# uncertaintyhub/chsimpy

Measured on AMD Instinct MI355X. Metric: timesteps/sec at N=4096 fp64; achieved HBM GB/s vs MI355X peak, higher is better.
Workload: dtype f64; 1 GPU; N=4096 fp64 Cahn-Hilliard timestep loop (BASELINE.json configs[2] at N=4096), U_init = 0.875 + 0.00875*(PCG64(2023).random - 0.5), kappa_tilde=0.0002989112919661156, full_sim; N=4096, engine=fast, ensemble=single run

## Files before the change

### chsimpy_amd/csrc/chs_fast_core.h

```cpp
#pragma once
#include <hip/hip_runtime.h>
#include <type_traits>
#include "chs_cx.h"

template <typename T_, int N_, int G_, int THREADS_, int R0_, int RA_, int RB_, int RL_, int PAD1_, int PAD2_,
          int PADL_, int WPS_, int CT_ = THREADS_ / G_, int XPAIR_ = -1>
struct FCfg {
  using T = T_;
  using V = Cx<T_>;
  static constexpr int N = N_;
  static constexpr int M = N_ / 2;
  static constexpr int G = G_;
  static constexpr int E = M / G_;
  static constexpr int R0 = R0_, RA = RA_, RB = RB_, RL = RL_;
  static constexpr int R2 = RL_;
  static constexpr int S1 = R0_;
  static constexpr int S2A = R0_ * RA_;
  static constexpr int SL = R0_ * RA_ * RB_;
  static constexpr int S2 = SL;
  static constexpr int L1 = M / R0_;
  static constexpr int L2 = L1 / RA_;
  static constexpr int L3 = L2 / RB_;
  static constexpr int NP0 = E / (2 * R0_);
  static constexpr int NBA = E / RA_;
// ... 318 lines not shown
  }
}
template <class C, bool WR, int PART>
__device__ __forceinline__ void mv_a_out(typename C::V* z, typename C::T* scr, int l) {
#pragma unroll
  for (int ib = 0; ib < C::NBA; ++ib) {
    const int id = l + C::G * ib;
    const int kap = id % C::S1, mm = id / C::S1;
#pragma unroll
    for (int k = 0; k < C::RA; ++k) {
      if constexpr (C::RB > 1) xfer<C, WR, PART>(z[ib * C::RA + k], scr, (kap + C::S1 * k) * C::P2 + mm);
      else xfer<C, WR, PART>(z[ib * C::RA + k], scr, mm * C::PL + kap + C::S1 * k);
    }
  }
}
template <class C, bool WR, int PART>
__device__ __forceinline__ void mv_b_in(typename C::V* z, typename C::T* scr, int l) {
#pragma unroll
  for (int ib = 0; ib < C::NBB; ++ib) {
    const int id = l + C::G * ib;
    const int kap = id % C::S2A, mm = id / C::S2A;
#pragma unroll
    for (int j = 0; j < C::RB; ++j) xfer<C, WR, PART>(z[ib * C::RB + j], scr, kap * C::P2 + mm + C::L3 * j);
  }
}
template <class C, bool WR, int PART>
__device__ __forceinline__ void mv_b_out(typename C::V* z, typename C::T* scr, int l) {
#pragma unroll
  for (int ib = 0; ib < C::NBB; ++ib) {
    const int id = l + C::G * ib;
    const int kap = id % C::S2A, mm = id / C::S2A;
#pragma unroll
    for (int k = 0; k < C::RB; ++k) xfer<C, WR, PART>(z[ib * C::RB + k], scr, mm * C::PL + kap + C::S2A * k);
  }
}
template <class C, bool WR, int PART>
__device__ __forceinline__ void mv_last(typename C::V* z, typename C::T* scr, int l) {
#pragma unroll
  for (int q = 0; q < C::NP2; ++q) {
    int k1, k2; bool sp;
    Own<C>::last_pair(l, q, k1, k2, sp);
#pragma unroll
    for (int j = 0; j < C::RL; ++j) {
      xfer<C, WR, PART>(z[(q * 2 + 0) * C::RL + j], scr, j * C::PL + k1);
      xfer<C, WR, PART>(z[(q * 2 + 1) * C::RL + j], scr, j * C::PL + k2);
    }
  }
}

#define CHS_EXCHANGE(WRITER, READER)                                                   \
  do {                                                                                 \
    xsync<C>(); WRITER<C, true, 0>(z, scr, l); xsync<C>(); READER<C, false, 0>(z, scr, l);   \
    if constexpr (!C::PAIR) {                                                          \
      xsync<C>(); WRITER<C, true, 1>(z, scr, l); xsync<C>(); READER<C, false, 1>(z, scr, l); \
    }                                                                                  \
  } while (0)

template <class C, bool POW>
__device__ __forceinline__ void tw0_load(const typename C::T* tw0, int m, typename C::V* w ) {
  using T = typename C::T;
  if constexpr (!POW) {
#pragma unroll
    for (int k = 1; k < C::R0; ++k) w[k] = ldc<T>(tw0, (k - 1) * C::L1 + m);
  } else {
    w[1] = ldc<T>(tw0, m);
#pragma unroll
    for (int k = 2; k < C::R0; ++k) w[k] = cx_mul(w[k / 2], w[k - k / 2]);
  }
}

template <class C, bool TW0POW = false>
__device__ __forceinline__ void fwd_passes(typename C::V* z, typename C::T* scr, const FTables<typename C::T>& tb, int l) {
  using T = typename C::T;
  using V = typename C::V;
#pragma unroll
  for (int q = 0; q < C::NP0; ++q) {
    const int m1 = l + C::G * q;
#pragma unroll
    for (int b = 0; b < 2; ++b) {
      const int m = b ? (C::L1 - 1 - m1) : m1;
      V* r = z + (q * 2 + b) * C::R0;
      Dft<V, C::R0, false>::run(r);
      V w[C::R0];
      tw0_load<C, TW0POW>(tb.tw0, m, w);
#pragma unroll
      for (int k = 1; k < C::R0; ++k) r[k] = cx_mul(r[k], w[k]);
    }
  }
  if constexpr (C::RA > 1) {
    CHS_EXCHANGE(mv_pass0, mv_a_in);
    mid_fwd<C, C::S1, C::L2, C::RA, C::NBA>(z, tb.twa, l);
    if constexpr (C::RB > 1) {
      CHS_EXCHANGE(mv_a_out, mv_b_in);
      mid_fwd<C, C::S2A, C::L3, C::RB, C::NBB>(z, tb.twb, l);
      CHS_EXCHANGE(mv_b_out, mv_last);
    } else {
      CHS_EXCHANGE(mv_a_out, mv_last);
    }
  } else {
    CHS_EXCHANGE(mv_pass0, mv_last);
  }
#pragma unroll
  for (int q = 0; q < 2 * C::NP2; ++q) Dft<V, C::RL, false>::run(z + q * C::RL);
}

template <class C, bool TW0POW = false>
__device__ __forceinline__ void inv_passes(typename C::V* z, typename C::T* scr, const FTables<typename C::T>& tb, int l) {
  using T = typename C::T;
  using V = typename C::V;
#pragma unroll
  for (int q = 0; q < 2 * C::NP2; ++q) Dft<V, C::RL, true>::run(z + q * C::RL);
  if constexpr (C::RA > 1) {
    if constexpr (C::RB > 1) {
      CHS_EXCHANGE(mv_last, mv_b_out);
      mid_inv<C, C::S2A, C::L3, C::RB, C::NBB>(z, tb.twb, l);
      CHS_EXCHANGE(mv_b_in, mv_a_out);
    } else {
      CHS_EXCHANGE(mv_last, mv_a_out);
    }
    mid_inv<C, C::S1, C::L2, C::RA, C::NBA>(z, tb.twa, l);
    CHS_EXCHANGE(mv_a_in, mv_pass0);
  } else {
    CHS_EXCHANGE(mv_last, mv_pass0);
  }
#pragma unroll
  for (int q = 0; q < C::NP0; ++q) {
    const int m1 = l + C::G * q;
#pragma unroll
    for (int b = 0; b < 2; ++b) {
      const int m = b ? (C::L1 - 1 - m1) : m1;
      V* r = z + (q * 2 + b) * C::R0;
      V w[C::R0];
      tw0_load<C, TW0POW>(tb.tw0, m, w);
#pragma unroll
      for (int k = 1; k < C::R0; ++k) r[k] = cx_mulc(r[k], w[k]);
      Dft<V, C::R0, true>::run(r);
    }
  }
}

#ifndef CHS_RSTAMP
#define CHS_RSTAMP(I) do {} while (0)
#define CHS_RSTAMP1(I) do {} while (0)
#endif
struct NoFetch {};
__device__ __forceinline__ int fc_opaque(int x) {
  asm volatile("" : "+v"(x));
  __builtin_assume(x >= 0 && x < 8192);
  return x;
}

template <class C>
struct PreAll { static constexpr bool value = (C::E <= 8); };
template <class C, bool FWD, bool ADJ, bool PIPE_, class PRE, class F, class ST>
__device__ __forceinline__ void recombine(typename C::V* z, const FTables<typename C::T>& tb, int l, PRE&& pre, F&& f, ST&& st) {
  using T = typename C::T;
  using V = typename C::V;
  constexpr bool PREALL = PreAll<C>::value;
  constexpr bool PIPE = PIPE_ && !PREALL;
  constexpr int R2 = C::R2, N = C::N, M = C::M, H = R2 / 2;
  const V zero = cx_make(T(0), T(0));
#pragma unroll
  for (int q = 0; q < C::NP2; ++q) {
    V* r1 = z + (q * 2 + 0) * R2;
    V* r2 = z + (q * 2 + 1) * R2;
    const int kap = l + C::G * q;
    bool has_special = false;
    if (q == 0) has_special = (C::G < 64) || (__builtin_amdgcn_readfirstlane(l) == 0);
    if (!has_special) {
      SlotTw<T> wn;
      const int id0[5] = {kap, N - kap, M - kap, M + kap, kap};
      decltype(pre(0, id0)) pn;
      [[maybe_unused]] SlotTw<T> wv[PREALL ? R2 : 1];
      [[maybe_unused]] decltype(pre(0, id0)) pv[PREALL ? R2 : 1];
      if constexpr (PIPE) {
        wn = slot_tw<T>(tb, kap);
        pn = pre(q * R2 * 4, id0);
      }
      if constexpr (PREALL) {
#pragma unroll
        for (int k = 0; k < R2; ++k) {
          const int kk = kap + C::S2 * k;
          wv[k] = slot_tw<T>(tb, kk);
          const int idc[5] = {kk, N - kk, M - kk, M + kk, kk};
          pv[k] = pre((q * R2 + k) * 4, idc);
        }
      }
      CHS_RSTAMP1(0);
#pragma unroll
      for (int k = 0; k < R2; ++k) {
        if (k == 1) CHS_RSTAMP1(1);
        if (k == 4) CHS_RSTAMP1(2);
        const int kk = kap + C::S2 * k;
        if constexpr (PREALL) {
          wn = wv[k]; pn = pv[k];
        } else if (!PIPE) {
          wn = slot_tw<T>(tb, kk);
          const int idc[5] = {kk, N - kk, M - kk, M + kk, kk};
          pn = pre((q * R2 + k) * 4, idc);
        }
        const SlotTw<T> w = wn;
        const auto pc = pn;
        V Ya = zero, Yb = zero;
        if constexpr (FWD) slot_fwd<T>(r1[k], r2[R2 - 1 - k], w, Ya, Yb);
        const int idx[5] = {kk, N - kk, M - kk, M + kk, kk};
        f((q * R2 + k) * 4, idx, Ya, Yb, true, pc);
        if (PIPE && k + 1 < R2) {
          const int kn = fc_opaque(kap) + C::S2 * (k + 1);
          wn = slot_tw<T>(tb, kn);
          const int idn[5] = {kn, N - kn, M - kn, M + kn, kn};
          pn = pre((q * R2 + k + 1) * 4, idn);
        }
        st((q * R2 + k) * 4, idx, Ya, Yb, true);
        if constexpr (ADJ) slot_adj<T>(Ya, Yb, w, r1[k], r2[R2 - 1 - k]);
      }
      CHS_RSTAMP1(3);
    } else {
      const bool sp = (kap == 0);
      auto sel = [&](V a, V b) { return cx_make(sp ? cx_re(a) : cx_re(b), sp ? cx_im(a) : cx_im(b)); };
      auto kk_of = [&](int k) {
        const int kk_s = (k == 0) ? C::S2 : ((k < H) ? C::S2 * k : C::S2 / 2 + C::S2 * (k - H));
        return sp ? kk_s : kap + C::S2 * k;
      };
      const int kk0 = kk_of(0);
      SlotTw<T> wn;
      const int o1 = PIPE ? (sp ? 0 : kk0) : kk0, o2 = PIPE ? (sp ? M / 2 : N - kk0) : N - kk0;
      const int o3 = PIPE ? (sp ? M : M - kk0) : M - kk0, o4 = PIPE ? (sp ? 3 * (M / 2) : M + kk0) : M + kk0;
      const int id0[5] = {o1, o2, o3, o4, (PIPE && sp) ? M + 1 : kk0};
      decltype(pre(0, id0)) pn;
      SlotTw<T> whp = SlotTw<T>();
      [[maybe_unused]] SlotTw<T> wv[PREALL ? R2 : 1];
      [[maybe_unused]] decltype(pre(0, id0)) pv[PREALL ? R2 : 1];
      [[maybe_unused]] SlotTw<T> w0v = SlotTw<T>();
      [[maybe_unused]] decltype(pre(0, id0)) p0v;
      if constexpr (PIPE) {
        wn = slot_tw<T>(tb, o1);
        pn = pre(q * R2 * 4, id0);
        if (sp) whp = slot_tw<T>(tb, M / 2);
      }
      if constexpr (PREALL) {
        if (sp) {
          const int ido[5] = {0, M / 2, M, 3 * (M / 2), M + 1};
          w0v = slot_tw<T>(tb, 0); whp = slot_tw<T>(tb, M / 2);
          p0v = pre(q * R2 * 4, ido);
        }
#pragma unroll
        for (int k = 0; k < R2; ++k) {
          const int kk = kk_of(k);
          wv[k] = slot_tw<T>(tb, kk);
          const int idc[5] = {kk, N - kk, M - kk, M + kk, kk};
          pv[k] = pre((q * R2 + k) * 4, idc);
        }
      }
      CHS_RSTAMP(0);
      if (sp) {
        const int idx[5] = {0, M / 2, M, 3 * (M / 2), M + 1};
        SlotTw<T> w0, wh;
        decltype(pre(0, id0)) p0;
        if constexpr (PREALL) {
          w0 = w0v; wh = whp; p0 = p0v;
        } else if constexpr (PIPE) {
          w0 = wn; wh = whp; p0 = pn;
        } else {
          w0 = slot_tw<T>(tb, 0); wh = slot_tw<T>(tb, M / 2);
          p0 = pre(q * R2 * 4, idx);
        }
        V Ya = zero, Yb = zero;
        if constexpr (FWD) {
          V a01, a23, b01, b23;
          slot_fwd<T>(r1[0], r1[0], w0, a01, a23);
          slot_fwd<T>(r1[H], r1[H], wh, b01, b23);
          Ya = cx_make(cx_re(a01), cx_re(b01));
          Yb = cx_make(cx_re(a23), cx_im(b01));
        }
        f(q * R2 * 4, idx, Ya, Yb, true, p0);
        st(q * R2 * 4, idx, Ya, Yb, true);
        if constexpr (ADJ) {
          V ga, gz;
          slot_adj<T>(cx_make(cx_re(Ya), T(0)), cx_make(cx_re(Yb), T(0)), w0, ga, gz);
          r1[0] = cx_add(ga, gz);
          slot_adj<T>(cx_make(cx_im(Ya), cx_im(Yb)), zero, wh, ga, gz);
          r1[H] = cx_add(ga, gz);
        }
      }
      CHS_RSTAMP(1);
#pragma unroll
      for (int k = 0; k < R2; ++k) {
        if (k == 1) CHS_RSTAMP(2);
        if (k == 4) CHS_RSTAMP(3);
        const int kk = kk_of(k);
        if constexpr (PREALL) {
          wn = wv[k]; pn = pv[k];
        } else if (!PIPE) {
          wn = slot_tw<T>(tb, kk);
          const int idc[5] = {kk, N - kk, M - kk, M + kk, kk};
          pn = pre((q * R2 + k) * 4, idc);
        }
        const SlotTw<T> w = wn;
        const auto pc = pn;
        V* a_n = &r1[k]; V* b_n = &r2[R2 - 1 - k];
        V* a_s = (k < H) ? &r1[k] : &r2[k - H];
        V* b_s = (k == 0) ? &r2[R2 - 1] : ((k < H) ? &r1[R2 - k] : &r2[R2 - 1 - (k - H)]);
        V Ya = zero, Yb = zero;
        if constexpr (FWD) slot_fwd<T>(sel(*a_s, *a_n), sel(*b_s, *b_n), w, Ya, Yb);
        const int idx[5] = {kk, N - kk, M - kk, M + kk, kk};
        const bool live = (k > 0) || !sp;
        f((q * R2 + k) * 4, idx, Ya, Yb, live, pc);
        if (PIPE && k + 1 < R2) {
          const int kap_o = fc_opaque(kap);
          const int kn = sp ? kk_of(k + 1) : kap_o + C::S2 * (k + 1);
          wn = slot_tw<T>(tb, kn);
          const int idn[5] = {kn, N - kn, M - kn, M + kn, kn};
          pn = pre((q * R2 + k + 1) * 4, idn);
        }
        st((q * R2 + k) * 4, idx, Ya, Yb, live);
        if constexpr (ADJ) {
          V na, nb;
          slot_adj<T>(Ya, Yb, w, na, nb);
          if (k == 0) {
            *a_n = sel(*a_n, na);
            *b_n = sel(*b_n, nb);
          } else {
            if (k < H) {
              *a_n = na;
            } else {
              *a_s = sel(na, *a_s);
              *a_n = sel(*a_n, na);
            }
            *b_s = sel(nb, *b_s);
            *b_n = sel(*b_n, nb);
          }
        }
      }
      CHS_RSTAMP(4);
    }
  }
}

template <class C>
__device__ __forceinline__ void pack_quads(const typename C::T q1[4], const typename C::T q2[4], int q, int j, typename C::V* z) {
  constexpr int R0 = C::R0;
  z[(q * 2 + 0) * R0 + j] = cx_make(q1[0], q1[2]);
  z[(q * 2 + 1) * R0 + j] = cx_make(q2[0], q2[2]);
  z[(q * 2 + 1) * R0 + (R0 - 1 - j)] = cx_make(q1[3], q1[1]);
  z[(q * 2 + 0) * R0 + (R0 - 1 - j)] = cx_make(q2[3], q2[1]);
}
template <class C>
__device__ __forceinline__ void unpack_quads(const typename C::V* z, int q, int j, typename C::T q1[4], typename C::T q2[4]) {
  constexpr int R0 = C::R0;
  q1[0] = cx_re(z[(q * 2 + 0) * R0 + j]); q1[2] = cx_im(z[(q * 2 + 0) * R0 + j]);
  q2[0] = cx_re(z[(q * 2 + 1) * R0 + j]); q2[2] = cx_im(z[(q * 2 + 1) * R0 + j]);
  q1[3] = cx_re(z[(q * 2 + 1) * R0 + (R0 - 1 - j)]); q1[1] = cx_im(z[(q * 2 + 1) * R0 + (R0 - 1 - j)]);
  q2[3] = cx_re(z[(q * 2 + 0) * R0 + (R0 - 1 - j)]); q2[1] = cx_im(z[(q * 2 + 0) * R0 + (R0 - 1 - j)]);
}
```

### chsimpy_amd/csrc/chs_fast_f64.hip

```cpp
#if !defined(CHS_STAMPS) || defined(CHS_FAST_UNITY_INCLUDE)
#include "chs_fast_kernels.h"

using F128 = FCfg<double, 128, 8, 64, 4, 4, 1, 4, 1, 0, 1, 2>;
using F256 = FCfg<double, 256, 16, 64, 4, 8, 1, 4, 1, 0, 1, 2>;
using F512 = FCfg<double, 512, 32, 128, 4, 4, 4, 4, 1, 1, 1, 2>;
using F512C = FCfg<double, 512, 32, 64, 4, 4, 4, 4, 1, 1, 1, 2, 4>;
using F1024 = FCfg<double, 1024, 64, 256, 4, 8, 4, 4, 2, 1, 4, 2>;
using F2048 = FCfg<double, 2048, 64, 256, 8, 16, 1, 8, 2, 0, 8, 2>;
using F2048C = F2048;
template <> struct ColLamSgpr<F2048C> { static constexpr bool value = false; };
#ifndef CHS_ROW_WPS
#define CHS_ROW_WPS 4
#endif
#ifndef CHS_ROW_THREADS
#define CHS_ROW_THREADS 256
#endif
#ifndef CHS_ROW_PADL
#define CHS_ROW_PADL 4
#endif
#ifndef CHS_F4096_CT
#define CHS_F4096_CT 4
#endif
#ifndef CHS_PAD1
#define CHS_PAD1 2
#endif
#ifndef CHS_PAD2
#define CHS_PAD2 1
#endif
#ifndef CHS_COL_PADL
#define CHS_COL_PADL 16
#endif
using F4096 = FCfg<double, 4096, 128, CHS_ROW_THREADS, 8, 4, 8, 8, CHS_PAD1, CHS_PAD2, CHS_ROW_PADL, CHS_ROW_WPS, CHS_F4096_CT>;
#ifndef CHS_F4096_ROW_TW_LDS
#define CHS_F4096_ROW_TW_LDS 3
#endif
template <> struct RowTwLds<F4096> { static constexpr int value = CHS_F4096_ROW_TW_LDS; };
#ifndef CHS_COL_WPS
#define CHS_COL_WPS 2
#endif
#ifndef CHS_COL_THREADS
#define CHS_COL_THREADS 256
#endif
using F4096C = FCfg<double, 4096, 128, CHS_COL_THREADS, 8, 4, 8, 8, CHS_PAD1, CHS_PAD2, CHS_COL_PADL, CHS_COL_WPS, CHS_F4096_CT>;
#ifndef CHS_F4096C_TW_LDS
#define CHS_F4096C_TW_LDS 2
#endif
template <> struct ColTwLds<F4096C> { static constexpr int value = CHS_F4096C_TW_LDS; };

#ifndef CHS_F8192_CT
#define CHS_F8192_CT 8
#endif
using F8192 = FCfg<double, 8192, 256, 512, 8, 8, 8, 8, 2, 1, 16, 4, CHS_F8192_CT>;
using F8192C = FCfg<double, 8192, 256, 512, 8, 8, 8, 8, 2, 1, 16, 2, CHS_F8192_CT>;
#ifndef CHS_F8192C_TW_LDS
#define CHS_F8192C_TW_LDS 2
#endif
template <> struct ColTwLds<F8192C> { static constexpr int value = CHS_F8192C_TW_LDS; };
template <> struct ColLamSgpr<F8192C> { static constexpr bool value = false; };
#ifndef CHS_F8192_ROW_TW_LDS
#define CHS_F8192_ROW_TW_LDS 3
#endif
template <> struct RowTwLds<F8192> { static constexpr int value = CHS_F8192_ROW_TW_LDS; };


bool chs_fast_bind_f64(int N, FastPlan* P) {
  switch (N) {
    case 128: bind<F128>(P); bind_batch<F128>(P); break;
    case 256: bind<F256>(P); bind_batch<F256>(P); break;
    case 512: bind<F512, F512C>(P); bind_batch<F512, F512C>(P); break;
    case 1024: bind<F1024>(P); bind_batch<F1024>(P); break;
    case 2048: bind<F2048, F2048C>(P); bind_batch<F2048, F2048C>(P); break;
    case 4096: bind<F4096, F4096C>(P); break;
    case 8192: bind<F8192, F8192C>(P); break;
    default: return false;
  }
  return true;
}
#endif
```

### chsimpy_amd/csrc/chs_fast_kernels.h

```cpp
#pragma once
#include <cmath>
#include <vector>
#include <cstdlib>

#include "chs_common.h"
#ifdef CHS_STAMPS
#define CHS_NSTAMP 12
#ifdef CHS_FAST_MAIN_TU
__device__ unsigned long long g_stamps[2][8192 * CHS_NSTAMP];
#endif
#define STAMP(K, I)                                                                         \
  do {                                                                                      \
    __builtin_amdgcn_sched_barrier(0);                                                      \
    unsigned long long t__;                                                                 \
    asm volatile("s_memtime %0\n\ts_waitcnt lgkmcnt(0)" : "=s"(t__)::"memory");            \
    __builtin_amdgcn_sched_barrier(0);                                                      \
    if (threadIdx.x == 0 && blockIdx.x < 8192) g_stamps[K][blockIdx.x * CHS_NSTAMP + (I)] = t__; \
  } while (0)
#define CHS_RSTAMP(I) do { if constexpr (PIPE) STAMP(1, 6 + (I)); } while (0)
#define CHS_RSTAMP1(I)                                                                      \
  do {                                                                                      \
    if constexpr (PIPE) {                                                                   \
      __builtin_amdgcn_sched_barrier(0);                                                    \
      unsigned long long t__;                                                               \
// ... 563 lines not shown
      double rs = 0.0;
      if (mine) {
#pragma unroll
        for (int e = 0; e < C::E; ++e) rs += (double)cx_re(z[e]) + (double)cx_im(z[e]);
      }
      const double rmean = block_sum_w(rs, red, wv, C::THREADS / 64) / (double)C::N;
      double ad = 0.0;
      if (mine) {
#pragma unroll
        for (int e = 0; e < C::E; ++e) ad += fabs((double)cx_re(z[e]) - rmean) + fabs((double)cx_im(z[e]) - rmean);
      }
      const double ra = block_sum_w(ad, red, wv, C::THREADS / 64) / (double)C::N;
      if (ra_blk && wv == 0 && chs_lane_id() == 0) partRa[0] = ra;
      __syncthreads();
    }
    const T RT = (T)dc.RT, BRT = (T)dc.BRT, B = (T)dc.B, A0 = (T)dc.A0, A1 = (T)dc.A1;
    const double mean = mean_u, thr = dc.threshold;
    double sE = 0.0, sPS = 0.0, s2 = 0.0;
    int cSA = 0;
    unsigned dom = 0;
    auto point = [&](T& u) {
      const T uinv = T(1) - u;
      const T lU = chs_log_unit_tab<T>(u, ltab, dom), lV = chs_log_unit_tab<T>(uinv, ltab, dom);
      sE += (double)chs_energy_from_logs_fast<T>(u, uinv, lU, lV, RT, B, A0, A1);
      sPS += fabs((double)u - mean);
      cSA += ((double)u < thr) ? 1 : 0;
      if constexpr (FUSE) {
        const T m = chs_mu_from_logs_fast<T>(u, uinv, lU, lV, RT, BRT, A0, A1);
        s2 += (double)m * (double)m;
        u = m;
        asm volatile("" : "+v"(u), "+v"(s2));
      }
      asm volatile("" : "+v"(sE), "+v"(sPS), "+v"(cSA), "+v"(dom));
    };
#pragma unroll
    for (int e = 0; e < C::E; ++e) {
      T a = cx_re(z[e]), b = cx_im(z[e]);
      point(a);
      point(b);
      z[e] = cx_make(a, b);
      __builtin_amdgcn_sched_barrier(0);
    }
    if (dom > (unsigned)(CHS_LOGTAB_N - 1)) sE = __builtin_nan("");
    const double acc[5] = {sE, sEdge, sPS, (double)cSA, s2};
    block_reduce_begin<5, FreshLane<C>::value>(acc, red, wv);
  }
  if constexpr (ADAPT) {
    constexpr int LDSB = C::C * C::SCR * (int)sizeof(T);
    constexpr int NH = (C::C == 1 || C::N * (int)sizeof(T) <= LDSB) ? 1 : 2;
    constexpr int JH = (C::R0 / 2) / NH;
    static_assert(!ADAPT || (FUSE && C::C <= 4 && (C::C == 1 || C::N * (int)sizeof(T) / NH <= LDSB) && (C::R0 / 2) % NH == 0),
                  "partial column sums need the scratch");
    const long long cs = st->computed_steps + 1;
    if (cs > 500 && (cs % 2) == 0) {
      const int lg = row_l<C>(wv, l);
      const int sub_a = row_sub<C>(wv, sub);
      T* prow = partColRows + (size_t)blockIdx.x * C::N;
      T* gl = reinterpret_cast<T*>(chs_dyn_lds);
      const T dmax = (T)dc.delt_max;
#pragma unroll
      for (int h = 0; h < NH; ++h) {
#pragma unroll
        for (int s = C::C - 1; s >= 0; --s) {
          __syncthreads();
          if (sub_a == s) {
#pragma unroll
            for (int q = 0; q < C::NP0; ++q) {
              const int m1 = lg + C::G * q, m2 = C::L1 - 1 - m1;
#pragma unroll
              for (int j = h * JH; j < (h + 1) * JH; ++j) {
                T q1[4], q2[4];
                unpack_quads<C>(z, q, j, q1, q2);
                const int c1 = 4 * (m1 + C::L1 * j), c2 = 4 * (m2 + C::L1 * j);
                const int o1 = c1 - h * (C::N / NH), o2 = c2 - h * (C::N / NH);
                T g1[4], g2[4];
#pragma unroll
                for (int e = 0; e < 4; ++e) {
                  g1[e] = chs_dt_integrand_fast(q1[e], dmax);
                  g2[e] = chs_dt_integrand_fast(q2[e], dmax);
                  if (s < C::C - 1) { g1[e] += gl[o1 + e]; g2[e] += gl[o2 + e]; }
                  if (s > 0) { gl[o1 + e] = g1[e]; gl[o2 + e] = g2[e]; }
                }
                if (s == 0) {
                  if constexpr (chs_grid_exceeds_cache(C::N, sizeof(T))) { store4_nt<T>(&prow[c1], g1); store4_nt<T>(&prow[c2], g2); }
                  else { store4<T>(&prow[c1], g1); store4<T>(&prow[c2], g2); }
                }
                __builtin_amdgcn_sched_barrier(0);
              }
            }
          }
        }
      }
      __syncthreads();
    }
  }
  if constexpr (DIAG && FUSE) STAMP(0, 4);
  if constexpr (FUSE) {
    __builtin_amdgcn_sched_barrier(0);
    T* scr_f = reinterpret_cast<T*>(chs_dyn_lds) + (size_t)row_sub<C>(wv, sub) * C::SCR;
    fwd_passes<C, RTW>(z, scr_f, tbp, row_l<C>(wv, l));
    if constexpr (DIAG && FUSE) STAMP(0, 5);
    __builtin_amdgcn_sched_barrier(0);
    const int lr = row_l<C>(wv, l), sr = row_sub<C>(wv, sub);
    const int rw = row_of_block<C>(blockIdx.x) + sr;
    recombine<C, true, false, false>(z, tb, lr, [](int, const int*) { return NoFetch{}; },
                              [](int, const int*, Cx<T>&, Cx<T>&, bool, NoFetch) {},
                              [&](int pbase, const int* idx, Cx<T>& Ya, Cx<T>& Yb, bool live) {
      if (live) {
        const T y[4] = {cx_re(Ya), cx_im(Ya), cx_re(Yb), cx_im(Yb)};
        row_store<C>(T1, rw, pbase, launder(lr), idx, y);
      }
    });
  }
  if constexpr (DIAG && FUSE) STAMP(0, 6);
  if constexpr (DIAG) {
    double out5[5];
    if (block_reduce_end<5, C::THREADS / 64>(red, out5, wv)) {
      double* p = partDiag + (size_t)blockIdx.x * 4;
      p[0] = out5[0]; p[1] = out5[1]; p[2] = out5[2]; p[3] = out5[3];
      if (FUSE) partMu[blockIdx.x] = out5[4];
    }
  }
}

template <class C>
struct ColStage {
  static constexpr int LINE = 4 * C::C;
  static constexpr int LP = LINE + 1;
  static constexpr int LINES = C::M / 4;
  static constexpr int ROWS = C::N / 2;
  static constexpr int ELEMS = LINES * LP;
  static constexpr int JR = C::R0 / 4;
  static constexpr int PW = (sizeof(typename C::T) == 4 && C::C % 4 == 0) ? 4 : ((C::C % 2 == 0) ? 2 : 1);
  static constexpr int PER = ROWS * C::C / (PW * C::THREADS);
  static constexpr int Q = C::CT / C::C;
  static_assert(C::R0 >= 4, "pass-0 radix must be >= 4");
  static_assert((ROWS * C::C) % (PW * C::THREADS) == 0, "the tile must split evenly over the threads");
  static __device__ __forceinline__ size_t goff(int rho, int f, int h) {
    const int row = f / C::C, c = f % C::C;
    return ((size_t)rho * ROWS + row) * C::CT + h * C::C + c;
  }
  static __device__ __forceinline__ int loff(int f) {
    const int row = f / C::C, c = f % C::C;
    return (row / 4) * LP + (row % 4) * C::C + c;
  }
};

template <class C>
struct ColTwLds { static constexpr int value = 1; };
template <class C>
struct ColLamSgpr { static constexpr bool value = true; };
template <class C>
struct ColLateStart { static constexpr bool value = (sizeof(typename C::T) == 4) || (C::N >= 4096); };
template <class C>
constexpr int col_tw_lds_elems() {
  if (ColTwLds<C>::value == 1) return 2 * ((C::R0 - 1) * C::L1 + (C::RA > 1 ? (C::RA - 1) * C::L2 : 0) + (C::RB > 1 ? (C::RB - 1) * C::L3 : 0));
  if (ColTwLds<C>::value == 2) return 2 * (C::L1 + (C::RA > 1 ? (C::RA - 1) * C::L2 : 0) + (C::RB > 1 ? (C::RB - 1) * C::L3 : 0));
  return 0;
}

template <class C>
constexpr int col_lds_elems() {
  return (C::C * C::SCR > ColStage<C>::ELEMS) ? C::C * C::SCR : ColStage<C>::ELEMS;
}

template <class C, int MODE, class... Batch>
__global__ __launch_bounds__(C::THREADS, C::WPS) void k_col(const typename C::T* __restrict__ Tin, typename C::T* __restrict__ Tout,
                                                typename C::T* __restrict__ hat, typename C::T* __restrict__ nat,
                                                FTables<typename C::T> tb, const double* __restrict__ lam,
                                                const double* __restrict__ sinsq, DevState* __restrict__ st,
                                                double* __restrict__ partE2, TailArgs ta, Batch... mem) {
  using T = typename C::T;
  using CS = ColStage<C>;
  if constexpr (sizeof...(Batch) != 0) {
    static_assert(MODE == MODE_STEP, "batches launch the step's column pass only");
    ConstBatchMember& m = batch_member(mem...);
    if (m.st->rows_written >= m.nsteps) return;
    Tin = (const T*)m.T1; Tout = (T*)m.T1; hat = (T*)m.hat; st = m.st; partE2 = m.partE2;
  }
  __shared__ double red[32];
  __shared__ int halted;
  constexpr bool LATE_HALT = (MODE == MODE_STEP) && ColLateStart<C>::value;
  if constexpr (MODE == MODE_STEP && !LATE_HALT) {
    if (threadIdx.x == 0) halted = st->halt;
    __syncthreads();
    if (halted) return;
  } else if constexpr (MODE != MODE_STEP) {
    if (st->halt) return;
  }
  if constexpr (MODE == MODE_STEP) STAMP(1, 0);
  T* lds = reinterpret_cast<T*>(chs_dyn_lds);
  int bid = blockIdx.x;
  if constexpr (MODE == MODE_STEP) {
    if (ta.enabled) {
      const bool at_end = !ta.gate;
      if (bid == (at_end ? (int)gridDim.x - 1 : 0)) {
        if constexpr (LATE_HALT) {
          if (threadIdx.x == 0) halted = st->halt;
          __syncthreads();
          if (halted) return;
        }
        step_tail_body<C::THREADS>(ta, st, reinterpret_cast<double*>(chs_dyn_lds));
        return;
      }
      if (!at_end) bid -= 1;
    }
  }
  const int l = threadIdx.x % C::G, sub = threadIdx.x / C::G;
  int ct, hh;
  if constexpr (CS::Q == 1) {
    ct = bid; hh = 0;
  } else {
    const int xcd = bid & 7, j = bid >> 3;
    ct = xcd + 8 * (j / CS::Q); hh = j % CS::Q;
  }
  if constexpr (MODE == MODE_STEP) {
    if (ta.reverse) ct = C::N / C::CT - 1 - ct;
  }
  const int kcp = ct * C::CT + hh * C::C + sub;
  const int kc = col_coef<C>(kcp);
  T* scr = lds + (size_t)sub * C::SCR;
  typename C::V z[C::E];
  FTables<T> tbp = tb;
  constexpr bool TW0POW = (MODE == MODE_STEP) && (ColTwLds<C>::value == 2);
  constexpr bool TW_SPLIT = LATE_HALT && (ColTwLds<C>::value != 0);
  constexpr int TW_N0 = TW0POW ? 2 * C::L1 : 2 * (C::R0 - 1) * C::L1;
  constexpr int TW_NM = col_tw_lds_elems<C>() - TW_N0;
  constexpr int TW_I0 = (TW_N0 + 2 * C::THREADS - 1) / (2 * C::THREADS), TW_IM = (TW_NM + 2 * C::THREADS - 1) / (2 * C::THREADS);
  using TwPair = typename std::conditional<sizeof(T) == 8, double2, float2>::type;
  [[maybe_unused]] TwPair tws_a[TW_SPLIT ? TW_I0 : 1], tws_b[TW_SPLIT ? (TW_IM > 0 ? TW_IM : 1) : 1];
  if constexpr (TW_SPLIT) {
#pragma unroll
    for (int i = 0; i < TW_I0; ++i) {
      const int e = 2 * ((int)threadIdx.x + i * C::THREADS);
      if (e < TW_N0) tws_a[i] = *reinterpret_cast<const TwPair*>(tb.tw0 + e);
    }
#pragma unroll
    for (int i = 0; i < TW_IM; ++i) {
      const int e = 2 * ((int)threadIdx.x + i * C::THREADS);
      if (e < TW_NM) tws_b[i] = *reinterpret_cast<const TwPair*>(tb.twa + e);
    }
    T* ltw = lds + col_lds_elems<C>();
    tbp.tw0 = ltw;
    tbp.twa = ltw + TW_N0;
    tbp.twb = tbp.twa + (C::RA > 1 ? 2 * (C::RA - 1) * C::L2 : 0);
  }
  if constexpr (MODE == MODE_STEP && ColTwLds<C>::value != 0 && !TW_SPLIT) {
    T* ltw = lds + col_lds_elems<C>();
    constexpr int N0 = TW0POW ? 2 * C::L1 : 2 * (C::R0 - 1) * C::L1;
    constexpr int NM = col_tw_lds_elems<C>() - N0;
    auto cp = [&](T* dst, const T* src, int n) {
      for (int i = 2 * threadIdx.x; i < n; i += 2 * C::THREADS) {
        if constexpr (sizeof(T) == 8) *reinterpret_cast<double2*>(dst + i) = *reinterpret_cast<const double2*>(src + i);
        else *reinterpret_cast<float2*>(dst + i) = *reinterpret_cast<const float2*>(src + i);
      }
    };
    cp(ltw, tb.tw0, N0);
    cp(ltw + N0, tb.twa, NM);
    tbp.tw0 = ltw;
    tbp.twa = ltw + N0;
    tbp.twb = tbp.twa + (C::RA > 1 ? 2 * (C::RA - 1) * C::L2 : 0);
  }
  T* hcol = hat + (size_t)kcp * C::N;
  T* hout = (MODE == MODE_STEP && nat != nullptr) ? nat + (size_t)kcp * C::N : hcol;
  double lam1 = st->lam1, lam2 = st->lam2;
  const int kc_u = (C::G >= 64) ? __builtin_amdgcn_readfirstlane(kc) : kc;
  const double lc = lam[kc_u];
  const double sqc = (MODE == MODE_STEP) ? sinsq[2 * kc_u + 1] : 0.0;
  constexpr bool HAT_STREAM = chs_grid_exceeds_cache(C::N, sizeof(T));
  constexpr bool HAT_NT_LD = HAT_STREAM, HAT_NT_ST = HAT_STREAM;
  struct Fetched64 { double2 ls[4]; Cx<T> h01, h23; };
  struct Fetched32 { float4 la, sa; Cx<T> h01, h23; };
  using Fetched = typename std::conditional<sizeof(T) == 8, Fetched64, Fetched32>::type;
  auto fetch = [&](int pbase, const int* idx) {
    Fetched p;
    if constexpr (sizeof(T) == 8) {
#pragma unroll
      for (int t = 0; t < 4; ++t) p.ls[t] = reinterpret_cast<const double2*>(sinsq)[idx[t]];
    } else {
      p.la = reinterpret_cast<const float4*>(tb.lam4)[idx[4]];
      p.sa = reinterpret_cast<const float4*>(tb.sin4)[idx[4]];
    }
    const int hp = hat_pair_index<C>(pbase, fc_opaque(l));
    p.h01 = ldc_hint<T, HAT_NT_LD>(hcol, hp);
    p.h23 = ldc_hint<T, HAT_NT_LD>(hcol, hp + C::G);
    return p;
  };
  if constexpr (MODE != MODE_INV_NATURAL && MODE != MODE_INV_NATIVE) {
    const T* tile = Tin + (size_t)ct * C::N * C::CT;
    constexpr int PER = CS::PER;
    constexpr int PW = CS::PW;
    T stage[2][PW * PER];
    auto request = [&](int rho) {
#pragma unroll
      for (int i = 0; i < PER; ++i) {
        const int f = PW * (threadIdx.x + i * C::THREADS);
        const T* src = tile + CS::goff(rho, f, hh);
        constexpr bool NT = (MODE == MODE_FWD_NATIVE);
        if constexpr (PW == 1) {
          stage[rho][i] = NT ? __builtin_nontemporal_load(src) : *src;
        } else if constexpr (PW == 4) {
          chs_f4v v;
          if constexpr (NT) v = __builtin_nontemporal_load(reinterpret_cast<const chs_f4v*>(src));
          else v = *reinterpret_cast<const chs_f4v*>(src);
          stage[rho][4 * i] = v.x; stage[rho][4 * i + 1] = v.y; stage[rho][4 * i + 2] = v.z; stage[rho][4 * i + 3] = v.w;
        } else if constexpr (sizeof(T) == 8) {
          if constexpr (NT) {
            const chs_d2v v = __builtin_nontemporal_load(reinterpret_cast<const chs_d2v*>(src));
            stage[rho][2 * i] = v.x; stage[rho][2 * i + 1] = v.y;
          } else {
            const double2 v = *reinterpret_cast<const double2*>(src);
            stage[rho][2 * i] = v.x; stage[rho][2 * i + 1] = v.y;
          }
        } else if constexpr (NT) {
          const chs_f2v v = __builtin_nontemporal_load(reinterpret_cast<const chs_f2v*>(src));
          stage[rho][2 * i] = v.x; stage[rho][2 * i + 1] = v.y;
        } else {
          const float2 v = *reinterpret_cast<const float2*>(src);
          stage[rho][2 * i] = v.x; stage[rho][2 * i + 1] = v.y;
        }
      }
    };
    request(0);
    if constexpr (TW_SPLIT) {
      T* ltw = lds + col_lds_elems<C>();
#pragma unroll
      for (int i = 0; i < TW_I0; ++i) {
        const int e = 2 * ((int)threadIdx.x + i * C::THREADS);
        if (e < TW_N0) *reinterpret_cast<TwPair*>(ltw + e) = tws_a[i];
      }
#pragma unroll
      for (int i = 0; i < TW_IM; ++i) {
        const int e = 2 * ((int)threadIdx.x + i * C::THREADS);
        if (e < TW_NM) *reinterpret_cast<TwPair*>(ltw + TW_N0 + e) = tws_b[i];
      }
    }
    if constexpr (LATE_HALT) {
      if (threadIdx.x == 0) halted = st->halt;
    }
#pragma unroll
    for (int rho = 0; rho < 2; ++rho) {
      __syncthreads();
      if constexpr (LATE_HALT) {
        if (rho == 0 && halted) return;
      }
#pragma unroll
      for (int i = 0; i < PER; ++i) {
        const int f = PW * (threadIdx.x + i * C::THREADS);
        const int lo = CS::loff(f);
#pragma unroll
        for (int e = 0; e < PW; ++e) lds[lo + e] = stage[rho][PW * i + e];
      }
      if (rho == 0) request(1);
      __syncthreads();
#pragma unroll
      for (int q = 0; q < C::NP0; ++q) {
        const int m1 = l + C::G * q, m2 = C::L1 - 1 - m1;
#pragma unroll
        for (int jj = 0; jj < CS::JR; ++jj) {
          const int j = rho * CS::JR + jj;
          T q1[4], q2[4];
#pragma unroll
          for (int e = 0; e < 4; ++e) {
            q1[e] = lds[(m1 + C::L1 * jj) * CS::LP + e * C::C + sub];
            q2[e] = lds[(m2 + C::L1 * jj) * CS::LP + e * C::C + sub];
          }
          pack_quads<C>(q1, q2, q, j, z);
        }
      }
    }
    __syncthreads();
    if constexpr (MODE == MODE_STEP) STAMP(1, 1);
    fwd_passes<C, TW0POW>(z, scr, tbp, l);
    if constexpr (MODE == MODE_STEP) STAMP(1, 2);
    if constexpr (MODE == MODE_STEP) {
      if (ta.gate) {
        if (gate_wait(st, ta.seq, ta.gate_spins, red, lam1, lam2)) return;
      }
    }
  }

  double e2 = 0.0;
  constexpr bool MEAN_NOW = !PreAll<C>::value;
  [[maybe_unused]] T h00 = T(0);
  constexpr bool FWD = (MODE != MODE_INV_NATURAL && MODE != MODE_INV_NATIVE);
  constexpr bool ADJ = (MODE == MODE_STEP || MODE == MODE_INV_NATURAL || MODE == MODE_INV_NATIVE);
  [[maybe_unused]] v2f e2v = {0.0f, 0.0f};
  if constexpr (MODE == MODE_STEP) {
    if constexpr (ColLamSgpr<C>::value) {
      auto uni = [](double x) {
        const long long b = __double_as_longlong(x);
        const unsigned lo = (unsigned)__builtin_amdgcn_readfirstlane((int)(b & 0xffffffffll));
        const unsigned hi = (unsigned)__builtin_amdgcn_readfirstlane((int)(b >> 32));
        return __longlong_as_double((long long)(((unsigned long long)hi << 32) | lo));
      };
      lam1 = uni(lam1); lam2 = uni(lam2);
    }
    [[maybe_unused]] const float lam1f = (float)lam1, lam2f = (float)lam2, lcf = (float)lc, sqcf = (float)sqc;
    auto spec_f =
      [&](int pbase, const int*, Cx<T>& Ya, Cx<T>& Yb, bool live, const Fetched& p) {
        if constexpr (sizeof(T) == 8) {
          T y[4] = {cx_re(Ya), cx_im(Ya), cx_re(Yb), cx_im(Yb)};
          const T hold[4] = {cx_re(p.h01), cx_im(p.h01), cx_re(p.h23), cx_im(p.h23)};
#pragma unroll
          for (int t = 0; t < 4; ++t) {
            const T h = chs_spectral<T>(hold[t], y[t], p.ls[t].x, lc, lam1, lam2);
            y[t] = h;
            const double term = (double)h * (double)h * (p.ls[t].y + sqc);
            e2 += live ? term : 0.0;
            if constexpr (MEAN_NOW) { if (pbase + t == 0 && live && l == 0 && kc == 0) st->meanU = (double)h / (double)C::N; }
            else if (pbase + t == 0 && live) h00 = h;
          }
          asm volatile("" : "+v"(e2));
          Ya = cx_make(y[0], y[1]); Yb = cx_make(y[2], y[3]);
        } else {
          auto upd = [&](v2f hold, v2f y, v2f lamr, v2f sr) {
            const v2f leig = lamr + lcf;
            const v2f CHeig = __builtin_elementwise_fma(lam2f * leig, leig, v2f{1.0f, 1.0f});
            const v2f rhs = __builtin_elementwise_fma(lam1f * leig, y, hold);
            v2f r;
            r.x = __builtin_amdgcn_rcpf(CHeig.x); r.y = __builtin_amdgcn_rcpf(CHeig.y);
            const v2f q = rhs * r;
            const v2f rho = __builtin_elementwise_fma(-CHeig, q, rhs);
            const v2f h = __builtin_elementwise_fma(rho, r, q);
            v2f term = (h * h) * (sr + sqcf);
            if (!live) term = v2f{0.0f, 0.0f};
            e2v += term;
            return h;
          };
          Ya = upd(p.h01, Ya, v2f{p.la.x, p.la.y}, v2f{p.sa.x, p.sa.y});
          Yb = upd(p.h23, Yb, v2f{p.la.z, p.la.w}, v2f{p.sa.z, p.sa.w});
          if constexpr (MEAN_NOW) { if (pbase == 0 && live && l == 0 && kc == 0) st->meanU = (double)Ya.x / (double)C::N; }
          else if (pbase == 0 && live) h00 = Ya.x;
        }
      };
    auto spec_st =
      [&](int pbase, const int*, Cx<T>& Ya, Cx<T>& Yb, bool live) {
        if (live) {
          const int hp = hat_pair_index<C>(pbase, fc_opaque(l));
          stc_hint<T, HAT_NT_ST>(hout, hp, Ya);
          stc_hint<T, HAT_NT_ST>(hout, hp + C::G, Yb);
        }
      };
    recombine<C, true, true, true>(z, tb, l, fetch, spec_f, spec_st);
    if constexpr (sizeof(T) == 4) e2 = (double)e2v.x + (double)e2v.y;
  } else {
    recombine<C, FWD, ADJ, false>(z, tb, l, [](int, const int*) { return NoFetch{}; },
                           [&](int pbase, const int* idx, Cx<T>& Ya, Cx<T>& Yb, bool live, NoFetch) {
      [[maybe_unused]] const int hp = hat_pair_index<C>(pbase, l);
      if constexpr (MODE == MODE_FWD_NATIVE) {
        if (live) { stc<T>(hcol, hp, Ya); stc<T>(hcol, hp + C::G, Yb); }
      } else if constexpr (MODE == MODE_INV_NATIVE) {
        Ya = ldc<T>(hcol, hp); Yb = ldc<T>(hcol, hp + C::G);
      } else {
        T y[4] = {cx_re(Ya), cx_im(Ya), cx_re(Yb), cx_im(Yb)};
#pragma unroll
        for (int t = 0; t < 4; ++t) {
          const int kr = idx[t];
          if constexpr (MODE == MODE_FWD_NATURAL) {
            if (live) nat[(size_t)kr * C::N + kc] = y[t];
          } else {
            y[t] = nat[(size_t)kr * C::N + kc];
          }
        }
        if constexpr (MODE != MODE_FWD_NATURAL) { Ya = cx_make(y[0], y[1]); Yb = cx_make(y[2], y[3]); }
      }
    }, [](int, const int*, Cx<T>&, Cx<T>&, bool) {});
  }
  if constexpr (MODE == MODE_STEP) STAMP(1, 5);
  if constexpr (MODE == MODE_STEP && !MEAN_NOW) {
    if (l == 0 && kc == 0) st->meanU = (double)h00 / (double)C::N;
  }
  if constexpr (MODE == MODE_STEP) STAMP(1, 3);
  if constexpr (ADJ) {
    inv_passes<C, TW0POW>(z, scr, tbp, l);
    if constexpr (MODE == MODE_STEP) STAMP(1, 4);
    T* tile = Tout + (size_t)ct * C::N * C::CT;
#pragma unroll
    for (int rho = 0; rho < 2; ++rho) {
      __syncthreads();
#pragma unroll
      for (int q = 0; q < C::NP0; ++q) {
        const int m1 = l + C::G * q, m2 = C::L1 - 1 - m1;
#pragma unroll
        for (int jj = 0; jj < CS::JR; ++jj) {
          const int j = rho * CS::JR + jj;
          T q1[4], q2[4];
          unpack_quads<C>(z, q, j, q1, q2);
#pragma unroll
          for (int e = 0; e < 4; ++e) {
            lds[(m1 + C::L1 * jj) * CS::LP + e * C::C + sub] = q1[e];
            lds[(m2 + C::L1 * jj) * CS::LP + e * C::C + sub] = q2[e];
          }
        }
      }
      __syncthreads();
#pragma unroll
      for (int i = 0; i < CS::PER; ++i) {
        const int f = CS::PW * (launder((int)threadIdx.x) + i * C::THREADS);
        const int lo = CS::loff(f);
        T* dst = tile + CS::goff(rho, f, hh);
        if constexpr (CS::PW == 1) {
          *dst = lds[lo];
        } else if constexpr (CS::PW == 4) {
          chs_f4v v; v.x = lds[lo]; v.y = lds[lo + 1]; v.z = lds[lo + 2]; v.w = lds[lo + 3];
          *reinterpret_cast<chs_f4v*>(dst) = v;
        } else {
          const T a = lds[lo], b = lds[lo + 1];
          if constexpr (sizeof(T) == 8) *reinterpret_cast<double2*>(dst) = make_double2(a, b);
          else *reinterpret_cast<float2*>(dst) = make_float2(a, b);
        }
      }
    }
  }
  if constexpr (MODE == MODE_STEP) {
    const double acc1[1] = {e2};
    double tot1[1];
    block_sum_store<1, C::THREADS / 64>(acc1, red, tot1);
    if (threadIdx.x == 0) partE2[bid] = tot1[0];
  }
}

enum { ROW_INV_PLAIN = 0, ROW_INV_DIAG = 1, ROW_INV_FUSED = 2, ROW_INV_FUSED_ADAPT = 3 };
enum { ROW_FWD_PLAIN = 0, ROW_FWD_POINTWISE = 1 };

struct FastPlan {
  int N, G, R0, RA, RB, RL, threads, col_tiles;
  void* tables = nullptr;
  size_t off_tw0, off_twa, off_twb, off_wp, off_t1, off_t2, off_lam4 = 0, off_sin4 = 0;
  int (*row_fwd)(Engine*, const void*, void*, int) = nullptr;
  int (*row_fwd2)(Engine*, const void*, void*, void*) = nullptr;
  int (*row_inv)(Engine*, int, const void*, void*, void*) = nullptr;
  int (*col)(Engine*, int, const void*, void*, void*, void*) = nullptr;
  int (*init)(Engine*) = nullptr;
  int (*init_batch)() = nullptr;
  int (*col_batch)(Engine* E0, hipStream_t s, const BatchMember* mem, int B, int reverse) = nullptr;
  int (*row_inv_batch)(Engine* E0, hipStream_t s, const BatchMember* mem, int B, bool fuse) = nullptr;
  int col_threads = 0;
};

template <typename T>
static FTables<T> get_tables(Engine* E) {
  FastPlan* P = (FastPlan*)E->dTw;
  const T* base = (const T*)P->tables;
  FTables<T> tb;
  tb.tw0 = base + P->off_tw0; tb.twa = base + P->off_twa; tb.twb = base + P->off_twb; tb.wp = base + P->off_wp;
  tb.t1 = base + P->off_t1; tb.t2 = base + P->off_t2;
  tb.lam4 = base + P->off_lam4; tb.sin4 = base + P->off_sin4;
  return tb;
}

template <class C, class CC = C>
struct Launch {
  using T = typename C::T;
  static constexpr size_t row_lds = (size_t)C::C * C::SCR * sizeof(T) + CHS_LOGTAB_N * 16 + (size_t)row_tw_lds_elems<C>() * sizeof(T);
  static constexpr bool ADAPT_OK = (C::C <= 4) && (C::C == 1 || (size_t)C::N * sizeof(T) / 2 <= row_lds) && (C::R0 % 4 == 0);
  static constexpr size_t col_lds = ((size_t)col_lds_elems<CC>() + (size_t)col_tw_lds_elems<CC>()) * sizeof(T);
  static_assert(C::N == CC::N && C::CT == CC::CT, "row/column configs must agree on the tile layout");

  template <class K>
  static int set_lds(K kernel, size_t bytes) {
    CHS_HIP(hipFuncSetAttribute((const void*)kernel, hipFuncAttributeMaxDynamicSharedMemorySize, (int)bytes));
    return CHS_OK;
  }
  static int init(Engine* E) {
    (void)E;
    int rc;
    if ((rc = set_lds(k_row_fwd<C, true>, row_lds))) return rc;
    if ((rc = set_lds(k_row_fwd<C, false>, row_lds))) return rc;
    if ((rc = set_lds(k_row_fwd2<C>, row_lds))) return rc;
    if ((rc = set_lds(k_row_inv<C, false, false>, row_lds))) return rc;
    if ((rc = set_lds(k_row_inv<C, true, false>, row_lds))) return rc;
    if ((rc = set_lds(k_row_inv<C, true, true>, row_lds))) return rc;
    if constexpr (ADAPT_OK) {
      if ((rc = set_lds(k_row_inv<C, true, true, true>, row_lds))) return rc;
    }
    E->adaptOk = ADAPT_OK;
    if ((rc = set_lds(k_col<CC, MODE_STEP>, col_lds))) return rc;
    if ((rc = set_lds(k_col<CC, MODE_FWD_NATIVE>, col_lds))) return rc;
    if ((rc = set_lds(k_col<CC, MODE_FWD_NATURAL>, col_lds))) return rc;
    if ((rc = set_lds(k_col<CC, MODE_INV_NATURAL>, col_lds))) return rc;
    if ((rc = set_lds(k_col<CC, MODE_INV_NATIVE>, col_lds))) return rc;
    return CHS_OK;
  }
  static int row_fwd(Engine* E, const void* in, void* out, int mode) {
    const int grid = C::N / C::C;
    if (mode == ROW_FWD_POINTWISE)
      k_row_fwd<C, true><<<grid, C::THREADS, row_lds, E->stream>>>((const T*)in, (T*)out, get_tables<T>(E), E->dc, E->dState,
                                                            E->dPartMu);
    else
      k_row_fwd<C, false><<<grid, C::THREADS, row_lds, E->stream>>>((const T*)in, (T*)out, get_tables<T>(E), E->dc, E->dState,
                                                             E->dPartMu);
    CHS_HIP(hipGetLastError());
    return CHS_OK;
  }
  static int row_fwd2(Engine* E, const void* in, void* ta, void* t1) {
    k_row_fwd2<C><<<C::N / C::C, C::THREADS, row_lds, E->stream>>>((const T*)in, (T*)ta, (T*)t1, get_tables<T>(E), E->dc,
// ... 124 lines not shown
```

Before: 4934 timesteps/s.

## Park half the column recombine operands in LDS to raise column kernel occupancy

Adds a parking mechanism that spills the second half of each recombine slot pair from registers into the LDS staging area before the fused column recombine stage, reloading each operand only around the slot that uses it. It also raises the column kernel's waves-per-SIMD launch bound from 2 to 3 for the N=4096 f64 column config. The aim is to cut VGPR pressure so more workgroups can be resident and hide memory latency. The cost is extra LDS traffic and a barrier per tile, plus a compile-time check that three workgroups still fit in a CU's LDS.

Result: no change. 4971 timesteps/s, median of 6 (+0.7%).

```diff
diff --git a/chsimpy_amd/csrc/chs_fast_core.h b/chsimpy_amd/csrc/chs_fast_core.h
--- a/chsimpy_amd/csrc/chs_fast_core.h
+++ b/chsimpy_amd/csrc/chs_fast_core.h
@@ -494,13 +494,48 @@
 
 template <class C>
 struct PreAll { static constexpr bool value = (C::E <= 8); };
-template <class C, bool FWD, bool ADJ, bool PIPE_, class PRE, class F, class ST>
-__device__ __forceinline__ void recombine(typename C::V* z, const FTables<typename C::T>& tb, int l, PRE&& pre, F&& f, ST&& st) {
+
+template <class C>
+constexpr int park_elems() { return 2 * C::NP2 * C::R2 * C::THREADS; }
+template <class C, bool WR>
+__device__ __forceinline__ void park_xfer(typename C::V& v, typename C::T* park, int j) {
+  using Item = typename std::conditional<sizeof(typename C::T) == 8, double2, v2f>::type;
+  Item* p = reinterpret_cast<Item*>(park) + j * C::THREADS;
+  if constexpr (sizeof(typename C::T) == 8) {
+    if constexpr (WR) *p = make_double2(v.x, v.y);
+    else { const double2 t = *p; v.x = t.x; v.y = t.y; }
+  } else {
+    if constexpr (WR) *p = v; else v = *p;
+  }
+}
+template <class C, bool WR>
+__device__ __forceinline__ void park_all(typename C::V* z, typename C::T* park) {
+#pragma unroll
+  for (int q = 0; q < C::NP2; ++q) {
+#pragma unroll
+    for (int j = 0; j < C::R2; ++j) park_xfer<C, WR>(z[(q * 2 + 1) * C::R2 + j], park, q * C::R2 + j);
+  }
+}
+
+template <class C, bool FWD, bool ADJ, bool PIPE_, bool PARK = false, class PRE, class F, class ST>
+__device__ __forceinline__ void recombine(typename C::V* z, const FTables<typename C::T>& tb, int l, PRE&& pre, F&& f, ST&& st,
+                                          [[maybe_unused]] typename C::T* park = nullptr) {
   using T = typename C::T;
   using V = typename C::V;
   constexpr bool PREALL = PreAll<C>::value;
   constexpr bool PIPE = PIPE_ && !PREALL;
   constexpr int R2 = C::R2, N = C::N, M = C::M, H = R2 / 2;
+  static_assert(!PARK || (FWD && ADJ), "parking is for the in-place stage: operands read and written per slot");
+  [[maybe_unused]] auto park_item = [&](const V* p) {
+    const int i = (int)(p - z);
+    return ((i / R2) & 1) ? (i / (2 * R2)) * R2 + i % R2 : -1;
+  };
+  [[maybe_unused]] auto park_in = [&](V* p) {
+    if constexpr (PARK) { const int j = park_item(p); if (j >= 0) park_xfer<C, false>(*p, park, j); }
+  };
+  [[maybe_unused]] auto park_out = [&](V* p) {
+    if constexpr (PARK) { const int j = park_item(p); if (j >= 0) park_xfer<C, true>(*p, park, j); }
+  };
   const V zero = cx_make(T(0), T(0));
 #pragma unroll
   for (int q = 0; q < C::NP2; ++q) {
@@ -541,6 +576,7 @@
           const int idc[5] = {kk, N - kk, M - kk, M + kk, kk};
           pn = pre((q * R2 + k) * 4, idc);
         }
+        park_in(&r2[R2 - 1 - k]);
         const SlotTw<T> w = wn;
         const auto pc = pn;
         V Ya = zero, Yb = zero;
@@ -555,6 +591,7 @@
         }
         st((q * R2 + k) * 4, idx, Ya, Yb, true);
         if constexpr (ADJ) slot_adj<T>(Ya, Yb, w, r1[k], r2[R2 - 1 - k]);
+        park_out(&r2[R2 - 1 - k]);
       }
       CHS_RSTAMP1(3);
     } else {
@@ -643,6 +680,10 @@
         V* a_n = &r1[k]; V* b_n = &r2[R2 - 1 - k];
         V* a_s = (k < H) ? &r1[k] : &r2[k - H];
         V* b_s = (k == 0) ? &r2[R2 - 1] : ((k < H) ? &r1[R2 - k] : &r2[R2 - 1 - (k - H)]);
+        const bool in_as = (a_s != b_n), in_bs = (b_s != b_n) && (b_s != a_s);
+        park_in(b_n);
+        if (in_as) park_in(a_s);
+        if (in_bs) park_in(b_s);
         V Ya = zero, Yb = zero;
         if constexpr (FWD) slot_fwd<T>(sel(*a_s, *a_n), sel(*b_s, *b_n), w, Ya, Yb);
         const int idx[5] = {kk, N - kk, M - kk, M + kk, kk};
@@ -673,6 +714,9 @@
             *b_n = sel(*b_n, nb);
           }
         }
+        park_out(b_n);
+        if (in_as) park_out(a_s);
+        if (in_bs) park_out(b_s);
       }
       CHS_RSTAMP(4);
     }
diff --git a/chsimpy_amd/csrc/chs_fast_f64.hip b/chsimpy_amd/csrc/chs_fast_f64.hip
--- a/chsimpy_amd/csrc/chs_fast_f64.hip
+++ b/chsimpy_amd/csrc/chs_fast_f64.hip
@@ -36,7 +36,10 @@
 #endif
 template <> struct RowTwLds<F4096> { static constexpr int value = CHS_F4096_ROW_TW_LDS; };
 #ifndef CHS_COL_WPS
-#define CHS_COL_WPS 2
+#define CHS_COL_WPS 3
+#endif
+#ifndef CHS_F4096C_PARK
+#define CHS_F4096C_PARK 1
 #endif
 #ifndef CHS_COL_THREADS
 #define CHS_COL_THREADS 256
@@ -46,6 +49,9 @@
 #define CHS_F4096C_TW_LDS 2
 #endif
 template <> struct ColTwLds<F4096C> { static constexpr int value = CHS_F4096C_TW_LDS; };
+template <> struct ColPark<F4096C> { static constexpr bool value = (CHS_F4096C_PARK != 0); };
+static_assert(CHS_COL_WPS * ((Launch<F4096, F4096C>::col_lds + 32 * sizeof(double) + sizeof(int) + 1279) / 1280 * 1280) <= 160 * 1024,
+              "k_col<F4096C>: the resident workgroups the kernel is compiled for must fit the LDS of a CU");
 
 #ifndef CHS_F8192_CT
 #define CHS_F8192_CT 8
diff --git a/chsimpy_amd/csrc/chs_fast_kernels.h b/chsimpy_amd/csrc/chs_fast_kernels.h
--- a/chsimpy_amd/csrc/chs_fast_kernels.h
+++ b/chsimpy_amd/csrc/chs_fast_kernels.h
@@ -739,6 +739,8 @@
 struct ColLamSgpr { static constexpr bool value = true; };
 template <class C>
 struct ColLateStart { static constexpr bool value = (sizeof(typename C::T) == 4) || (C::N >= 4096); };
+template <class C>
+struct ColPark { static constexpr bool value = false; };
 template <class C>
 constexpr int col_tw_lds_elems() {
   if (ColTwLds<C>::value == 1) return 2 * ((C::R0 - 1) * C::L1 + (C::RA > 1 ? (C::RA - 1) * C::L2 : 0) + (C::RB > 1 ? (C::RB - 1) * C::L3 : 0));
@@ -1029,7 +1031,16 @@
           stc_hint<T, HAT_NT_ST>(hout, hp + C::G, Yb);
         }
       };
-    recombine<C, true, true, true>(z, tb, l, fetch, spec_f, spec_st);
+    if constexpr (ColPark<C>::value) {
+      static_assert(park_elems<C>() <= col_lds_elems<C>(), "the parked values must fit the staging / exchange area");
+      T* park = lds + 2 * (chs_wave_id() * 64 + chs_lane_id());
+      __syncthreads();
+      park_all<C, true>(z, park);
+      recombine<C, true, true, true, true>(z, tb, l, fetch, spec_f, spec_st, park);
+      park_all<C, false>(z, park);
+    } else {
+      recombine<C, true, true, true>(z, tb, l, fetch, spec_f, spec_st);
+    }
     if constexpr (sizeof(T) == 4) e2 = (double)e2v.x + (double)e2v.y;
   } else {
     recombine<C, FWD, ADJ, false>(z, tb, l, [](int, const int*) { return NoFetch{}; },
```
